# bibymaths/phoskintime

Measured on AMD Instinct MI355X. Metric: ODE-solve replicas/sec (32-state distributive, 14 tp), higher is better.
Workload: dtype f64

## Files before the change

### include/phoskin.h

```cpp
#ifndef PHOSKIN_H
#define PHOSKIN_H

#include <stdint.h>

#ifdef __cplusplus
extern "C" {
#endif

#define PK_VERSION 200

enum { PK_MODEL_DIST = 0, PK_MODEL_SUCC = 1, PK_MODEL_RAND = 2 };

enum {
  PK_METHOD_RODAS4 = 0,
  PK_METHOD_BDF2   = 1,
  PK_METHOD_RK4    = 2,
  PK_METHOD_LRP8   = 3,
  PK_METHOD_LRP12  = 5,
  PK_METHOD_DP5    = 4,
  PK_METHOD_ARK436 = 6,
  PK_METHOD_ROS34PW2 = 7
};

enum {
// ... 135 lines not shown
  const int32_t *p_prot, *t_prot; const double *obs_prot, *w_prot;
  const int32_t *p_rna, *t_rna;   const double *obs_rna, *w_rna;
  const int32_t *p_pho, *s_pho, *t_pho; const double *obs_pho, *w_pho;
  int32_t prot_base_idx, rna_base_idx, pho_base_idx;
} pk_loss_data;
typedef struct pk_loss pk_loss;
pk_loss* pk_network_loss_create(pk_ctx*, pk_net*, const pk_loss_data*, int T);
void     pk_network_loss_destroy(pk_loss*);
int      pk_network_objective_batch(pk_ctx*, pk_net*, pk_loss*, int64_t B, const double* Y, int T, int loss_mode,
                                    const double* x, int x_is_raw, const double* defaults, const double* lambdas, double fail_value,
                                    const int32_t* status, double* loss_sums, double* F);

int      pk_network_simulate_objective_batch(pk_ctx*, pk_net*, pk_loss*, int64_t B, const double* x, int x_is_raw, const double* y0,
                                             int y0_is_batched, const double* t_host, int T, const pk_solver_opts* opts, int loss_mode,
                                             const double* defaults, const double* lambdas, double fail_value, double* Y, int32_t* status,
                                             int32_t* n_steps, double* loss_sums, double* F);

int pk_loss_fn_batch_host(pk_ctx*, int combinatorial, int loss_mode, int64_t B, const double* Y, int T, int S, const pk_loss_data*,
                          const int32_t* prot_map, int N, double* loss_sums);

int pk_network_observables_batch(pk_ctx*, pk_net*, pk_loss*, int64_t B, const double* Y, int T, double eps, double* pred);

enum { PK_NET_METRIC_TOTAL_SIGNAL = 0, PK_NET_METRIC_MEAN = 1, PK_NET_METRIC_VARIANCE = 2, PK_NET_METRIC_L2_NORM = 3 };
int pk_network_simulate_measure_batch(pk_ctx*, pk_net*, pk_loss* lists, int64_t B, const double* x, int x_is_raw, const double* y0,
                                      int y0_is_batched, const double* t_host, int T, const pk_solver_opts* opts, double eps, int metric_id,
                                      double* Y, double* pred, double* metric, int32_t* status, int32_t* n_steps);

double pk_time_solve_protein_batch(pk_ctx*, int iters, int model, int n_sites, int64_t B,
                                   const double* theta, const double* y0, int y0_is_batched,
                                   const double* t, int T, const pk_solver_opts* opts,
                                   double* sol, double* flat, double* metric, int metric_id,
                                   int32_t* status, int32_t* n_steps);

double pk_measure_hbm_gbs(pk_ctx*, int64_t bytes, int iters);
double pk_measure_hbm_stream_gbs(pk_ctx*, int64_t bytes, int iters, int mode);
double pk_measure_fp64_fma_tflops(pk_ctx*, int iters);

#define PK_COMM_ID_BYTES 128
int pk_comm_unique_id(pk_ctx*, char* id_out );
int pk_comm_init(pk_ctx*, const char* id , int rank, int world);
int pk_comm_rank(pk_ctx*);
int pk_comm_world(pk_ctx*);
int pk_allgather_f64(pk_ctx*, const double* send, int64_t count, double* recv);
int pk_comm_destroy(pk_ctx*);

#ifdef __cplusplus
}
#endif
#endif
```

### phoskintime_amd/_capi.py

```python
from __future__ import annotations

import ctypes as C
import os
from pathlib import Path

_HERE = Path(__file__).resolve().parent
LIB_PATH = _HERE / "libphoskin_hip.so"

DIST, SUCC, RAND = 0, 1, 2
MODEL_IDS = {"distmod": DIST, "succmod": SUCC, "randmod": RAND}
MODEL_NAMES = {v: k for k, v in MODEL_IDS.items()}
METHOD_RODAS4, METHOD_BDF2, METHOD_RK4, METHOD_LRP8, METHOD_DP5, METHOD_LRP12, METHOD_ARK436, METHOD_ROS34PW2 = 0, 1, 2, 3, 4, 5, 6, 7
METHODS = {"rodas4": METHOD_RODAS4, "bdf2": METHOD_BDF2, "rk4": METHOD_RK4, "lrp8": METHOD_LRP8, "dp5": METHOD_DP5, "lrp12": METHOD_LRP12, "ark436": METHOD_ARK436, "ros34pw2": METHOD_ROS34PW2}
LINSOLVE_AUTO, LINSOLVE_DENSE, LINSOLVE_STRUCTURED = 0, 1, 2
LINSOLVES = {"auto": LINSOLVE_AUTO, "dense": LINSOLVE_DENSE, "structured": LINSOLVE_STRUCTURED}
KERNEL_AUTO, KERNEL_GROUP, KERNEL_TPR, KERNEL_WORKSPACE = 0, 1, 2, 3
KERNELS = {"auto": KERNEL_AUTO, "group": KERNEL_GROUP, "tpr": KERNEL_TPR, "workspace": KERNEL_WORKSPACE}
NORMS = {"default": 0, "max": 1, "rms": 2}
METRICS = {"total_signal": 0, "mean_activity": 1, "variance": 2, "dynamics": 3, "l2_norm": 4}
ST_NONFINITE, ST_MAXSTEPS, ST_HMIN = 1, 2, 4


class PhoskinLibraryError(RuntimeError):
    pass


class PhoskinError(RuntimeError):
    pass


class NetworkDesc(C.Structure):
    _fields_ = [("model", C.c_int32), ("N", C.c_int32), ("n_K", C.c_int32), ("total_sites", C.c_int32), ("n_grid", C.c_int32),
                ("offset_y", C.c_void_p), ("offset_s", C.c_void_p), ("n_sites", C.c_void_p),
                ("W_indptr", C.c_void_p), ("W_indices", C.c_void_p), ("W_data", C.c_void_p),
                ("TF_indptr", C.c_void_p), ("TF_indices", C.c_void_p), ("TF_data", C.c_void_p),
                ("tf_deg", C.c_void_p), ("driver_map", C.c_void_p), ("kin_grid", C.c_void_p), ("kin_Kmat", C.c_void_p)]


class LossData(C.Structure):
    _fields_ = [("n_prot", C.c_int32), ("n_rna", C.c_int32), ("n_pho", C.c_int32),
                ("p_prot", C.c_void_p), ("t_prot", C.c_void_p), ("obs_prot", C.c_void_p), ("w_prot", C.c_void_p),
                ("p_rna", C.c_void_p), ("t_rna", C.c_void_p), ("obs_rna", C.c_void_p), ("w_rna", C.c_void_p),
                ("p_pho", C.c_void_p), ("s_pho", C.c_void_p), ("t_pho", C.c_void_p), ("obs_pho", C.c_void_p), ("w_pho", C.c_void_p),
                ("prot_base_idx", C.c_int32), ("rna_base_idx", C.c_int32), ("pho_base_idx", C.c_int32)]


class SolverOpts(C.Structure):
    _fields_ = [("method", C.c_int32), ("linsolve", C.c_int32), ("rtol", C.c_double), ("atol", C.c_double),
                ("h0", C.c_double), ("rk4_h", C.c_double), ("max_steps", C.c_int32), ("clip_nonneg", C.c_int32),
                ("normalize", C.c_int32), ("stage_form", C.c_int32), ("kernel", C.c_int32), ("err_norm", C.c_int32)]


SYMBOLS = (
    "pk_version", "pk_create", "pk_create_error", "pk_destroy", "pk_last_error", "pk_set_stream", "pk_use_own_stream", "pk_synchronize", "pk_default_opts", "pk_workspace_stats",
    "pk_protein_n_states", "pk_protein_n_params", "pk_protein_flat_len",
    "pk_solve_protein_batch", "pk_solve_protein_sens_batch", "pk_protein_sens_available", "pk_rhs_protein_batch", "pk_jacobian_protein_batch", "pk_steady_state_protein_batch", "pk_morris_build_batch", "pk_morris_effects_batch", "pk_score_fit_batch",
    "pk_solve_protein_batch_host", "pk_solve_protein_sens_batch_host", "pk_rhs_protein_batch_host", "pk_jacobian_protein_batch_host",
    "pk_time_solve_protein_batch", "pk_measure_hbm_gbs", "pk_measure_hbm_stream_gbs", "pk_measure_fp64_fma_tflops",
    "pk_network_create", "pk_network_destroy", "pk_network_n_states", "pk_network_n_var",
    "pk_network_rhs_batch", "pk_network_jacobian_batch", "pk_network_unpack_batch", "pk_network_simulate_batch",
    "pk_network_loss_create", "pk_network_loss_destroy", "pk_network_objective_batch", "pk_network_simulate_objective_batch", "pk_network_observables_batch", "pk_network_simulate_measure_batch", "pk_frechet_batch", "pk_loss_fn_batch_host", "pk_network_resolve_method",
    "pk_network_workspace_bytes",
    "pk_comm_unique_id", "pk_comm_init", "pk_comm_rank", "pk_comm_world", "pk_allgather_f64", "pk_comm_destroy",
)

PK_OK, PK_ERR_ARG, PK_ERR_UNSUPPORTED, PK_ERR_HIP, PK_ERR_NOMEM = 0, -1, -2, -3, -4
NET_METRIC_TOTAL_SIGNAL, NET_METRIC_MEAN, NET_METRIC_VARIANCE, NET_METRIC_L2_NORM = 0, 1, 2, 3
NET_METRICS = {"total_signal": NET_METRIC_TOTAL_SIGNAL, "mean": NET_METRIC_MEAN, "variance": NET_METRIC_VARIANCE, "l2_norm": NET_METRIC_L2_NORM}

_lib = None


def load():
    global _lib
    if _lib is not None:
        return _lib
    import torch
    if not LIB_PATH.exists():
        raise PhoskinLibraryError(
            f"{LIB_PATH} not found: build it with `python -c 'import __graft_entry__ as g; g.build()'` "
            "(hipcc --offload-arch=gfx950). There is no CPU fallback.")
    try:
        lib = C.CDLL(str(LIB_PATH), mode=getattr(os, "RTLD_NOW", 2))
    except OSError as e:
        raise PhoskinLibraryError(f"cannot load {LIB_PATH}: {e}") from e
    vp, i32, i64, dbl = C.c_void_p, C.c_int, C.c_int64, C.c_double
    optp = C.POINTER(SolverOpts)
    lib.pk_version.restype = i32
    lib.pk_create.restype = vp; lib.pk_create.argtypes = [i32]
    lib.pk_create_error.restype = C.c_char_p; lib.pk_create_error.argtypes = []
# ... 24 lines not shown
    lib.pk_network_create.restype = vp; lib.pk_network_create.argtypes = [vp, C.POINTER(NetworkDesc)]
    lib.pk_network_destroy.restype = None; lib.pk_network_destroy.argtypes = [vp]
    lib.pk_network_n_states.restype = i32; lib.pk_network_n_states.argtypes = [vp]
    lib.pk_network_n_var.restype = i32; lib.pk_network_n_var.argtypes = [vp]
    for f in ("pk_network_rhs_batch", "pk_network_jacobian_batch"):
        getattr(lib, f).restype = i32; getattr(lib, f).argtypes = [vp, vp, i64, vp, i32, vp, i32, vp, i32, vp]
    lib.pk_network_simulate_batch.restype = i32
    lib.pk_network_simulate_batch.argtypes = [vp, vp, i64, vp, i32, vp, i32, vp, i32, optp, vp, vp, vp]
    lib.pk_network_loss_create.restype = vp; lib.pk_network_loss_create.argtypes = [vp, vp, C.POINTER(LossData), i32]
    lib.pk_network_loss_destroy.restype = None; lib.pk_network_loss_destroy.argtypes = [vp]
    lib.pk_network_objective_batch.restype = i32
    lib.pk_network_objective_batch.argtypes = [vp, vp, vp, i64, vp, i32, i32, vp, i32, vp, vp, dbl, vp, vp, vp]
    lib.pk_network_simulate_objective_batch.restype = i32
    lib.pk_network_simulate_objective_batch.argtypes = [vp, vp, vp, i64, vp, i32, vp, i32, vp, i32, optp, i32, vp, vp, dbl, vp, vp, vp, vp, vp]
    lib.pk_network_observables_batch.restype = i32
    lib.pk_network_observables_batch.argtypes = [vp, vp, vp, i64, vp, i32, dbl, vp]
    lib.pk_network_simulate_measure_batch.restype = i32
    lib.pk_network_simulate_measure_batch.argtypes = [vp, vp, vp, i64, vp, i32, vp, i32, vp, i32, optp, dbl, i32, vp, vp, vp, vp, vp]
    lib.pk_network_resolve_method.restype = i32; lib.pk_network_resolve_method.argtypes = [vp, optp]
    lib.pk_network_workspace_bytes.restype = i64; lib.pk_network_workspace_bytes.argtypes = [vp, vp, i64]
    lib.pk_loss_fn_batch_host.restype = i32
    lib.pk_loss_fn_batch_host.argtypes = [vp, i32, i32, i64, vp, i32, i32, C.POINTER(LossData), vp, i32, vp]
    lib.pk_network_unpack_batch.restype = i32; lib.pk_network_unpack_batch.argtypes = [vp, vp, i64, vp, vp]
    lib.pk_comm_unique_id.restype = i32; lib.pk_comm_unique_id.argtypes = [vp, C.c_char_p]
    lib.pk_comm_init.restype = i32; lib.pk_comm_init.argtypes = [vp, C.c_char_p, i32, i32]
    lib.pk_comm_rank.restype = i32; lib.pk_comm_rank.argtypes = [vp]
    lib.pk_comm_world.restype = i32; lib.pk_comm_world.argtypes = [vp]
    lib.pk_allgather_f64.restype = i32; lib.pk_allgather_f64.argtypes = [vp, vp, i64, vp]
    lib.pk_comm_destroy.restype = i32; lib.pk_comm_destroy.argtypes = [vp]
    lib.pk_score_fit_batch.restype = i32; lib.pk_score_fit_batch.argtypes = [vp, i64, vp, i32, vp, vp, i32, vp, vp]
    lib.pk_measure_hbm_gbs.restype = dbl; lib.pk_measure_hbm_gbs.argtypes = [vp, i64, i32]
    lib.pk_measure_hbm_stream_gbs.restype = dbl; lib.pk_measure_hbm_stream_gbs.argtypes = [vp, i64, i32, i32]
    lib.pk_measure_fp64_fma_tflops.restype = dbl; lib.pk_measure_fp64_fma_tflops.argtypes = [vp, i32]
    lib.pk_time_solve_protein_batch.restype = dbl
    lib.pk_time_solve_protein_batch.argtypes = [vp, i32] + solve_args[1:]
    _lib = lib
    return lib


def default_opts(**kw) -> SolverOpts:
    o = SolverOpts()
    load().pk_default_opts(C.byref(o))
    for k, v in kw.items():
        if v is None:
            continue
        if k == "method" and isinstance(v, str):
            v = METHODS[v]
        if k == "linsolve" and isinstance(v, str):
            v = LINSOLVES[v]
        if k == "kernel" and isinstance(v, str):
            v = KERNELS[v]
        if k == "err_norm" and isinstance(v, str):
            v = NORMS[v]
        if not hasattr(o, k):
            raise TypeError(f"unknown solver option {k!r}")
        setattr(o, k, v)
    return o


class Context:

    def __init__(self, device: int = 0):
        self.lib = load()
        self.device = int(device)
        self._h = self.lib.pk_create(self.device)
        if not self._h:
# ... 34 lines not shown
```

### phoskintime_amd/csrc/pk_capi.hip

```cpp
#include <hip/hip_runtime.h>
#include <cmath>
#include <cstdio>
#include <cstring>
#include <cstdlib>
#include <mutex>
#include <string>
#include "../../include/phoskin.h"
#include "pk_launch.hpp"
#include "pk_sens.hpp"

struct pk_arena {
  void* p = nullptr; size_t bytes = 0; long long allocs = 0;
};
struct pk_ctx {
  int device;
  hipStream_t own_stream;
  hipStream_t stream;
  std::string err;
  hipEvent_t ev0, ev1;
  pk_arena stage, scratch;
  void* pin = nullptr; size_t pin_bytes = 0; long long pin_allocs = 0;
  std::recursive_mutex mu;
  hipEvent_t scratch_ev = nullptr; bool scratch_used = false;
};
// ... 227 lines not shown
  }
  static const int level6_env = [] { const char* v = getenv("PK_RAND_LEVEL6"); return v ? atoi(v) : 0; }();
  if (model == PK_MODEL_RAND && n_sites == 6 && level6_env == 1 && o.method == PK_METHOD_LRP12 && !o.stage_form) {
    if (B > 0x7fffffffLL) return fail(c, PK_ERR_ARG, "batch too large for one launch");
    PK_HIP(c, hipSetDevice(c->device));
    PK_HIP(c, pk::launch_rand_level(a, c->stream));
    return PK_OK;
  }
  static const int parity56_env = [] { const char* v = getenv("PK_RAND_PARITY56"); return v ? atoi(v) : -1; }();
  if (model == PK_MODEL_RAND && ((n_sites == 6 && parity56_env != 0) || (n_sites == 5 && parity56_env == 1)) && o.method == PK_METHOD_LRP12 &&
      o.linsolve == PK_LINSOLVE_AUTO && !o.stage_form) {
    if (B > 0x7fffffffLL) return fail(c, PK_ERR_ARG, "batch too large for one launch");
    PK_HIP(c, hipSetDevice(c->device));
    PK_HIP(c, pk::launch_rand_parity(a, c->stream));
    return PK_OK;
  }
  const bool rand_fast = model == PK_MODEL_RAND && resolvent_method(o.method) && (o.linsolve == PK_LINSOLVE_AUTO || a.S > 64) && !o.stage_form;
  if (a.S > 64 && !rand_fast)
    return fail(c, PK_ERR_UNSUPPORTED, "randmod n_sites = 6 (S = 65): only method RODAS4 / LRP8 in resolvent form (the generic kernels hold one state per lane)");
  const int G = a.S > 64 ? 64 : group_width(a.S);
  const long long rpb = 256 / G;
  const long long nblk = (B + rpb - 1) / rpb;
  if (nblk > 0x7fffffffLL) return fail(c, PK_ERR_ARG, "batch too large for one launch");
  const bool structured = (o.linsolve != PK_LINSOLVE_DENSE) && (model != PK_MODEL_RAND);
  PK_HIP(c, hipSetDevice(c->device));
  dim3 grid((unsigned)nblk);
  static const int tpr_env_once = [] { const char* v = getenv("PK_TPR"); return v ? atoi(v) : -1; }();
  const int tpr_env = o.kernel == PK_KERNEL_GROUP ? 0 : o.kernel == PK_KERNEL_TPR ? 1 : tpr_env_once;
  const long long tpr_min = (model == PK_MODEL_SUCC) ? (n_sites <= 8 ? 16384 : 32768) : (model == PK_MODEL_RAND) ? 32768 : (n_sites <= 8 ? 32768 : 49152);
  const bool tpr = o.method == PK_METHOD_LRP12 && o.linsolve == PK_LINSOLVE_AUTO && !o.stage_form && pk::tpr_available(model, n_sites) &&
                   (tpr_env == 1 || (tpr_env != 0 && B >= tpr_min));
  if (tpr)
    PK_HIP(c, pk::launch_tpr(a, model, c->stream));
  else if (model == PK_MODEL_DIST && resolvent_method(o.method) && o.linsolve == PK_LINSOLVE_AUTO && !o.stage_form)
    pk::launch_dist_fast(a, o.method, c->stream);
  else if (rand_fast)
    pk::launch_rand_fast(a, o.method, c->stream);
  else
    kSolve[model][gidx(G)](a, o.method, structured, grid, c->stream);
  PK_HIP(c, hipGetLastError());
  return PK_OK;
}

int pk_rhs_protein_batch(pk_ctx* c, int model, int n_sites, int64_t B, const double* theta, const double* y, double* dydt) {
  if (!c) return PK_ERR_ARG;
  int rc = check_model(c, model, n_sites);
  if (rc) return rc;
  if (B < 0) return fail(c, PK_ERR_ARG, "B must be >= 0");
  if (B == 0) return PK_OK;
  if (!theta || !y || !dydt) return fail(c, PK_ERR_ARG, "null pointer");
  const int S = pk::n_states(model, n_sites), P = pk::n_params(model, n_sites), G = S > 64 ? 1 : group_width(S);
  const long long rpb = 256 / G, nblk = (S > 64 ? (B * S + 255) / 256 : (B + rpb - 1) / rpb);
  if (nblk > 0x7fffffffLL) return fail(c, PK_ERR_ARG, "batch too large for one launch");
  PK_HIP(c, hipSetDevice(c->device));
  dim3 grid((unsigned)nblk);
  if (S > 64 && model != PK_MODEL_RAND) pk::launch_chain_rhs_wide(model, theta, y, dydt, (long long)B, n_sites, S, P, c->stream);
  else if (S > 64) pk::launch_rand_rhs_wide(theta, y, dydt, (long long)B, n_sites, S, P, c->stream);
  else kRhs[model][gidx(G)](theta, y, dydt, (long long)B, n_sites, S, P, grid, c->stream);
  PK_HIP(c, hipGetLastError());
  return PK_OK;
}

int pk_jacobian_protein_batch(pk_ctx* c, int model, int n_sites, int64_t B, const double* theta, double* J) {
  if (!c) return PK_ERR_ARG;
  int rc = check_model(c, model, n_sites);
  if (rc) return rc;
  if (B < 0) return fail(c, PK_ERR_ARG, "B must be >= 0");
  if (B == 0) return PK_OK;
  if (!theta || !J) return fail(c, PK_ERR_ARG, "null pointer");
// ... 164 lines not shown
  if (!c) return PK_ERR_ARG;
  std::lock_guard<std::recursive_mutex> host_guard(c->mu);
  int rc = check_model(c, model, n_sites);
  if (rc) return rc;
  if (B < 0) return fail(c, PK_ERR_ARG, "B must be >= 0");
  if (B == 0) return PK_OK;
  if (!theta || !y || !dydt) return fail(c, PK_ERR_ARG, "null pointer");
  const size_t S = pk::n_states(model, n_sites), P = pk::n_params(model, n_sites);
  PK_HIP(c, hipSetDevice(c->device));
  HostCall h(c);
  const size_t o_th = h.add_in(theta, (size_t)B * P * 8), o_y = h.add_in(y, (size_t)B * S * 8), o_f = h.add_out(dydt, (size_t)B * S * 8);
  if ((rc = h.upload())) return rc;
  rc = pk_rhs_protein_batch(c, model, n_sites, B, h.dev<const double>(o_th), h.dev<const double>(o_y), h.dev<double>(o_f));
  if (rc) { (void)hipStreamSynchronize(c->stream); return rc; }
  return h.download();
}

int pk_jacobian_protein_batch_host(pk_ctx* c, int model, int n_sites, int64_t B, const double* theta, double* J) {
  if (!c) return PK_ERR_ARG;
  std::lock_guard<std::recursive_mutex> host_guard(c->mu);
  int rc = check_model(c, model, n_sites);
  if (rc) return rc;
  if (B < 0) return fail(c, PK_ERR_ARG, "B must be >= 0");
  if (B == 0) return PK_OK;
  if (!theta || !J) return fail(c, PK_ERR_ARG, "null pointer");
  const size_t S = pk::n_states(model, n_sites), P = pk::n_params(model, n_sites);
  PK_HIP(c, hipSetDevice(c->device));
  HostCall h(c);
  const size_t o_th = h.add_in(theta, (size_t)B * P * 8), o_J = h.add_out(J, (size_t)B * S * S * 8);
  if ((rc = h.upload())) return rc;
  rc = pk_jacobian_protein_batch(c, model, n_sites, B, h.dev<const double>(o_th), h.dev<double>(o_J));
  if (rc) { (void)hipStreamSynchronize(c->stream); return rc; }
  return h.download();
}

double pk_time_solve_protein_batch(pk_ctx* c, int iters, int model, int n_sites, int64_t B, const double* theta,
                                   const double* y0, int y0_is_batched, const double* t, int T,
                                   const pk_solver_opts* opts, double* sol, double* flat, double* metric, int metric_id,
                                   int32_t* status, int32_t* n_steps) {
  if (!c || iters < 1) return -1.0;
  if (hipSetDevice(c->device) != hipSuccess) return -1.0;
  if (hipEventRecord(c->ev0, c->stream) != hipSuccess) return -1.0;
  for (int i = 0; i < iters; ++i) {
    int rc = pk_solve_protein_batch(c, model, n_sites, B, theta, y0, y0_is_batched, t, T, opts, sol, flat, metric, metric_id, status, n_steps);
    if (rc) return (double)rc;
  }
  if (hipEventRecord(c->ev1, c->stream) != hipSuccess) return -1.0;
  if (hipEventSynchronize(c->ev1) != hipSuccess) { c->err = "hipEventSynchronize failed"; return -1.0; }
  float ms = 0.f;
  if (hipEventElapsedTime(&ms, c->ev0, c->ev1) != hipSuccess) return -1.0;
  return (double)ms / iters;
}

}

namespace pk {
__global__ __launch_bounds__(256) void score_fit_kernel(const double* __restrict__ theta, const int P, const double* __restrict__ target,
                                                        const double* __restrict__ pred, const int N, const long long B,
                                                        const double alpha, const double beta, const double gamma, const double delta,
                                                        const double mu, double* __restrict__ out) {
  const long long b = (long long)blockIdx.x * 4 + (threadIdx.x >> 6);
  if (b >= B) return;
  const int lane = threadIdx.x & 63;
  const double* pb = pred + b * N;
  double s1 = 0.0, s2 = 0.0;
  for (int k = lane; k < N; k += 64) { const double r = fabs(target[k] - pb[k]) / (double)N; s1 += r; s2 = __builtin_fma(r, r, s2); }
// ... 26 lines not shown
```

### phoskintime_amd/csrc/pk_dist_fast.hpp

```cpp
#pragma once
#include "pk_solve_kernel.hpp"

namespace pk {

template <int RPL, bool RES = false>
struct Stg {
  double s[RPL];
  double R, P;
};
template <int RPL>
struct Stg<RPL, true> {
  double s[RPL];
};
template <int RPL, bool RES>
__device__ __forceinline__ void trk_axpy(Stg<RPL, RES>& acc, const double a, const Stg<RPL, RES>& u) {
#pragma unroll
  for (int j = 0; j < RPL; ++j) acc.s[j] = __builtin_fma(a, u.s[j], acc.s[j]);
  if constexpr (!RES) {
    acc.R = __builtin_fma(a, u.R, acc.R);
    acc.P = __builtin_fma(a, u.P, acc.P);
  }
}
template <int RPL, bool RES>
__device__ __forceinline__ Stg<RPL, RES> trk_scale(const double a, const Stg<RPL, RES>& u) {
// ... 30 lines not shown
  __host__ __device__ static __forceinline__ bool normalize(const SolveArgs& A) { return A.normalize != 0; }
  __host__ __device__ static __forceinline__ bool flat(const SolveArgs& A) { return A.flat != nullptr; }
  __host__ __device__ static __forceinline__ bool sol(const SolveArgs& A) { return A.sol != nullptr; }
  __host__ __device__ static __forceinline__ int mclass(const SolveArgs& A) { return dist_metric_class(A); }
  static bool matches(const SolveArgs&) { return true; }
};
using DistSolSum = DistFixed<true, false, false, true, PK_DM_SUM>;
using DistSolOnly = DistFixed<true, false, false, true, PK_DM_NONE>;
using DistFlatOnly = DistFixed<true, false, true, false, PK_DM_NONE>;

template <int RPL, int MC, bool RES = false> constexpr int dist_fast_slots() {
  return MC == PK_DM_FULL ? 3 * RPL + (RES ? 4 : 6) : MC == PK_DM_SUM ? 2 * RPL + 1 : 2 * RPL;
}

template <int RPL, bool PARK, int NT> struct Parked;
template <int RPL, int NT> struct Parked<RPL, false, NT> {
  double v[3 * RPL + 6];
  __device__ __forceinline__ explicit Parked(double*) {}
  template <int K> __device__ __forceinline__ double get() const { return v[K]; }
  template <int K> __device__ __forceinline__ void set(double x) { v[K] = x; }
  __device__ __forceinline__ void fence() {}
};
template <int RPL, int NT> struct Parked<RPL, true, NT> {
  typedef __attribute__((address_space(3))) double lds_double;
  lds_double* base;
  __device__ __forceinline__ explicit Parked(double* lds) : base((lds_double*)lds + threadIdx.x) {}
  template <int K> __device__ __forceinline__ double get() const { return base[K * NT]; }
  template <int K> __device__ __forceinline__ void set(double x) { base[K * NT] = x; }
  __device__ __forceinline__ void fence() { asm volatile("" : "+v"(base)); }
};
template <int RPL, bool PARK, int NT = 256, class CFG = DistAny, bool RES = false>
constexpr size_t dist_fast_lds_bytes() { return PARK ? (size_t)(dist_fast_slots<RPL, CFG::SLOT_MC, RES>() + RPL) * NT * sizeof(double) : 0; }

template <int G, int RPL, int METHOD, bool PARK = false, int MINB = (PARK ? 2 : 1), int NT = 256, class CFG = DistAny, bool RES = false>
__global__ __launch_bounds__(NT, MINB) void dist_fast_kernel(const SolveArgs A) {
  using Tab = ResolventTab<METHOD>;
  using Vec = Stg<RPL, RES>;
  extern __shared__ __align__(16) double park_lds[];
  Parked<RPL, PARK, NT> pk(park_lds);
  static_assert(dist_fast_lds_bytes<RPL, PARK, 64, CFG, RES>() * 4 * MINB <= 160 * 1024, "parked slots exceed the CU's LDS at this occupancy");
  constexpr int MCS = CFG::SLOT_MC;
  constexpr int NSL = dist_fast_slots<RPL, MCS, RES>(), FB = 3 * RPL + (RES ? 0 : 2);
  constexpr int K_SR = 0, K_DG = RPL, K_PS = 2 * RPL, K_PR = 3 * RPL, K_PP = 3 * RPL + 1, K_M1 = (MCS == PK_DM_FULL ? FB : 2 * RPL),
                K_M2 = FB + 1, K_MD = FB + 2, K_SH = FB + 3, K_Y = NSL;
  constexpr int RPB = NT / G;
  const int lane = lane_id();
  const int l = threadIdx.x & (G - 1);
  const long long rep = (long long)blockIdx.x * RPB + (threadIdx.x / G);
  if (rep >= A.B) return;
  const int n = A.n_sites, S = A.S, T = A.T;
  const int mclass = CFG::mclass(A);
  const double* __restrict__ th = A.theta + rep * A.P;

  const double cA = th[0], cB = th[1], cC = th[2];
  const bool isR = RES && l == 0, isP = RES && l == 1;
  const double w0 = isR ? cC : 1.0, k3 = isR ? cA : 0.0;
  double lsum = 0.0;
  static_for<RPL>([&](auto jc) {
    constexpr int j = decltype(jc)::value;
    const int i = l + G * j - (RES ? 2 : 0);
    const bool ok = i >= 0 && i < n;
    const double sr = ok ? th[4 + i] : 0.0;
    double dg = ok ? 1.0 + th[4 + n + i] : 1.0;
    if constexpr (RES && j == 0) dg = isR ? cB : isP ? -cC : dg;
    pk.template set<K_SR + j>(sr);
    pk.template set<K_DG + j>(dg);
    lsum += sr;
  });
  const double Dsum = th[3] + gsum<G>(lsum, lane);
  auto sites_only = [&](const double (&s)[RPL]) {
// ... 101 lines not shown
            const double dR = vR - prevR, dP = vP - prevP;
            mdyn = __builtin_fma(dR, dR, mdyn); mdyn = __builtin_fma(dP, dP, mdyn);
          }
          pk.template set<K_PR>(vR); pk.template set<K_PP>(vP);
        }
        pk.template set<K_M2>(m2); pk.template set<K_MD>(mdyn);
      }
    }
  };
  auto finish = [&](const int status, const int acc, const int rej) {
    if (mclass != PK_DM_NONE) {
      const double L = 2.0 * T + (double)T * n;
      const double tot = gsum<G>(pk.template get<K_M1>(), lane);
      double m = tot;
      if (A.metric_id == PK_METRIC_MEAN_ACTIVITY) m = tot / L;
      if constexpr (MCS == PK_DM_FULL) if (mclass == PK_DM_FULL) {
        const double m2 = pk.template get<K_M2>(), mdyn = pk.template get<K_MD>(), shift = pk.template get<K_SH>();
        switch (A.metric_id) {
          case PK_METRIC_VARIANCE: { const double q = gsum<G>(m2, lane); const double ms = tot / L - shift; m = q / L - ms * ms; } break;
          case PK_METRIC_DYNAMICS: m = gsum<G>(mdyn, lane); break;
          default: { const double q = gsum<G>(m2, lane); m = sqrt(fmax(q + 2.0 * shift * tot - L * shift * shift, 0.0)); } break;
        }
      }
      if (l == 0) A.metric[rep] = m;
    }
    if (l == 0) {
      if (A.status) A.status[rep] = status;
      if (A.n_steps) { A.n_steps[2 * rep] = acc; A.n_steps[2 * rep + 1] = rej; }
    }
  };

  emit(0, y, std::false_type{});
  int status = PK_ST_OK, nacc = 0;
  if (T < 2) { finish(status, 0, 0); return; }

  const double rtol = A.rtol, atol = A.atol;
  auto q = [&](double e, double ya, double yb) { return fabs(e) * approx_rcp(__builtin_fma(rtol, fmax(fabs(ya), fabs(yb)), atol)); };
  auto group_max = [&](const Vec& num, const Vec& a, const Vec& b) {
    auto mx = [](double p, double r) { return (p > r || p != p) ? p : r; };
    double m;
    if constexpr (RES) m = q(num.s[0], a.s[0], b.s[0]); else m = mx(q(num.R, a.R, b.R), q(num.P, a.P, b.P));
#pragma unroll
    for (int j = (RES ? 1 : 0); j < RPL; ++j) m = mx(m, q(num.s[j], a.s[j], b.s[j]));
    return gmax<G>(m, lane);
  };
  auto err_norm = [&](const Vec& e, const Vec& y, const Vec& yn) {
    constexpr int X = RES ? 0 : 2;
    double r[RPL + X];
    if constexpr (!RES) { r[0] = q(e.R, y.R, yn.R); r[1] = q(e.P, y.P, yn.P); }
    static_for<RPL>([&](auto jc) {
      constexpr int j = decltype(jc)::value;
      r[X + j] = q(e.s[j], y.s[j], yn.s[j]);
    });
    double m = tree_max(r);
    if (any_nan(r)) m = __builtin_inf();
    return gmax_num<G>(m, lane);
  };
  auto rhs_of = [&](const Vec& Y, const double sg) {
    Vec f;
    if constexpr (RES) {
      const double Rb = bcast<G, 0>(Y.s[0]), Pb = bcast<G, 1>(Y.s[0]);
      static_for<RPL>([&](auto jc) {
        constexpr int j = decltype(jc)::value;
        const double sr = pk.template get<K_SR + j>(), dg = pk.template get<K_DG + j>();
        if constexpr (j == 0) f.s[0] = __builtin_fma(isP ? -Dsum : sr, Pb, __builtin_fma(-dg, isP ? Rb : Y.s[0], isP ? sg : k3));
        else f.s[j] = __builtin_fma(sr, Pb, -dg * Y.s[j]);
      });
// ... 89 lines not shown
      for (int j = 0; j < RPL; ++j) u.s[j] = __builtin_fma(cw[j], xP, t[j]);
      u.R = xR; u.P = xP;
    }
    return u;
  };

  bool after_reject = false;
  auto state_bad = [&]() {
    double rows[RPL];
#pragma unroll
    for (int j = 0; j < RPL; ++j) rows[j] = y.s[j];
    if constexpr (PARK) {
      pk.fence();
      static_for<RPL>([&](auto jc) { constexpr int j = decltype(jc)::value; rows[j] = pk.template get<K_Y + j>(); });
    }
    bool b;
    if constexpr (RES) b = ((isR || isP) && nonfinite(rows[0])) || nonfinite(sites_only(rows));
    else b = (nonfinite(y.R)) || (nonfinite(y.P)) || (nonfinite(site_sum<G>(rows, lane)));
    return gmax<G>(b ? 1.0 : 0.0, lane);
  };
  auto coef_bad = [&]() {
    if constexpr (RES) {
      long long r2 = rep;
      asm volatile("" : "+v"(r2));
      const double* t2 = A.theta + r2 * A.P;
      return (nonfinite(t2[0])) || (nonfinite(t2[1])) || (nonfinite(t2[2]));
    } else return (nonfinite(cA)) || (nonfinite(cB)) || (nonfinite(cC));
  };
  int nsec = 0;
  __builtin_amdgcn_s_waitcnt(0x0F70);
  while (true) {
    bool nonfin = false;
    while (true) {
      const double tnx = A.t[k + 1 < T ? k + 1 : T - 1];
      const bool over = (CFG::LITERAL ? nacc + nsec : nsec) >= A.max_steps;
      const bool last = (tc + 1.0001 * h >= te);
      const double hs = last ? te - tc : ((tc + 2.0 * h > te) ? 0.5 * (te - tc) : h);
      if (over || !(hs > 1e-14 * fmax(fabs(tc), 1e-3))) { status |= over ? PK_ST_MAXSTEPS : PK_ST_HMIN; break; }
      if constexpr (PARK) {
        pk.fence();
        static_for<RPL>([&](auto jc) { constexpr int j = decltype(jc)::value; y.s[j] = pk.template get<K_Y + j>(); });
      }
      factor(Tab::GAM * hs);

      Vec z;
      {
        Vec r = y;
        if constexpr (RES) r.s[0] = __builtin_fma(qq, k3, y.s[0]); else r.R = __builtin_fma(qq, cA, y.R);
        z = solve(r);
        trk_axpy(z, -1.0, y);
      }
      Vec yn = y; trk_axpy(yn, Tab::B[0] / Tab::GAM, z);
      Vec u6;
      static_for<Tab::NS - 1>([&](auto kc) {
        constexpr int kk = 1 + decltype(kc)::value;
        constexpr double bk = Tab::B[kk] / Tab::GAM, ek = Tab::E[kk] / Tab::GAM;
        z = solve(z);
        trk_axpy(yn, bk, z);
        if constexpr (kk == 1) u6 = trk_scale(ek, z); else trk_axpy(u6, ek, z);
      });

      double err;
      if constexpr (CFG::LITERAL) err = group_max(u6, y, yn); else err = err_norm(u6, y, yn);
      const bool acc = (err <= 1.0);
      if constexpr (PARK) {
        if (acc) {
// ... 18 lines not shown
          continue;
        }
      } else {
        ++nsec;
        if (__builtin_expect(err != err || err > 1e300, 0)) { after_reject = true; h = 0.1 * hs; nonfin = true; break; }
      }
      double fac = root_q(err, Tab::Q) * (1.0 / 0.9);
      fac = fmax(1.0 / 6.0, fmin(5.0, fac));
      double hnew = hs * fast_rcp(fac);
      const bool land = acc && last;
      if constexpr (CFG::LITERAL) { nacc += acc ? 1 : 0; nsec += acc ? 0 : 1; }
      else nacc += (int)acc;
      if (acc && after_reject) hnew = fmin(hnew, hs);
      after_reject = !acc;
      if constexpr (CFG::LITERAL) tc = land ? te : (acc ? tc + hs : tc);
      h = (land && hs < h) ? fmax(hnew, h) : hnew;
      if (land) {
        if constexpr (!CFG::LITERAL) tc = te;
        te = tnx;
        asm volatile("" : "+v"(te));
        emit(k, y, std::false_type{});
        ++k;
      }
      if (k >= T) break;
    }
    if (CFG::LITERAL || !nonfin) break;
    if (state_bad() != 0.0 || coef_bad() || (nonfinite(Dsum)) || (nonfinite(Scw))) {
      status |= PK_ST_NONFINITE; break;
    }
  }
  const int nrej = CFG::LITERAL ? nsec : nsec - nacc;
  if (status != PK_ST_OK)
    for (; k < T; ++k) emit(k, y, std::true_type{});
  finish(status, nacc, nrej);
}

}
```

### phoskintime_amd/csrc/pk_dist_fast12.hpp

```cpp
#pragma once
#include "pk_dist_fast.hpp"
#include "pk_launch.hpp"

namespace pk {

template <int G, int RPL, bool PARK, int NT, class CFG, bool RES>
static void launch_cfg(const SolveArgs& a, hipStream_t st) {
  const long long rpb = NT / G;
  const long long nblk = (a.B + rpb - 1) / rpb;
  constexpr size_t lds = dist_fast_lds_bytes<RPL, PARK, NT, CFG, RES>();
  auto kern = dist_fast_kernel<G, RPL, PK_METHOD_LRP12, PARK, (PARK ? 2 : 1), NT, CFG, RES>;
  if constexpr (lds > 48 * 1024) {
    static const bool once = [kern] {
      (void)hipFuncSetAttribute((const void*)kern, hipFuncAttributeMaxDynamicSharedMemorySize, (int)lds);
      return true;
    }();
    (void)once;
  }
  hipLaunchKernelGGL(kern, dim3((unsigned)nblk), dim3(NT), lds, st, a);
}

template <int G, int RPL, bool PARK, int NT, bool RES>
static void launch_nt(const SolveArgs& a, hipStream_t st) {
  if (DistSolSum::matches(a)) launch_cfg<G, RPL, PARK, NT, DistSolSum, RES>(a, st);
  else if (DistSolOnly::matches(a)) launch_cfg<G, RPL, PARK, NT, DistSolOnly, RES>(a, st);
  else if (DistFlatOnly::matches(a)) launch_cfg<G, RPL, PARK, NT, DistFlatOnly, RES>(a, st);
  else launch_cfg<G, RPL, PARK, NT, DistAny, RES>(a, st);
}

void launch_dist_fast12_resident(const SolveArgs& a, bool wg256, hipStream_t st);

}
```

### phoskintime_amd/csrc/pk_inst_dist_fast12.hip

```cpp
#include "pk_dist_fast12.hpp"
#include <cstdio>
#include <cstdlib>
#include <cstring>

namespace pk {

template <int G, int RPL>
static void launch_plain(const SolveArgs& a, hipStream_t st) { launch_nt<G, RPL, false, 256, false>(a, st); }

template <int G, int RPL>
static void launch_parked(const SolveArgs& a, hipStream_t st) { launch_nt<G, RPL, true, 64, false>(a, st); }

void launch_dist_fast12(const SolveArgs& a, hipStream_t st) {
  const int n = a.n_sites;
  static const bool force84 = getenv("PK_DIST_LAYOUT") && !strcmp(getenv("PK_DIST_LAYOUT"), "8x4");
  static const bool wg256 = getenv("PK_DIST_LAYOUT") && !strcmp(getenv("PK_DIST_LAYOUT"), "wg256");
  static const bool shadow = getenv("PK_DIST_LAYOUT") && !strcmp(getenv("PK_DIST_LAYOUT"), "shadow");
  const int slots = n <= 32 ? 4 * ((n + 3) / 4) : 8 * ((n + 7) / 8);
  if (!shadow && !(force84 && n > 16 && n <= 32) && n >= 1 && slots >= n + 2) { launch_dist_fast12_resident(a, wg256, st); return; }
  if (n <= 4) launch_plain<4, 1>(a, st);
  else if (n <= 8) launch_plain<4, 2>(a, st);
  else if (n <= 12) launch_plain<4, 3>(a, st);
  else if (n <= 16) launch_plain<4, 4>(a, st);
  else if (n <= 32 && force84) launch_plain<8, 4>(a, st);
  else if (n <= 20) launch_parked<4, 5>(a, st);
  else if (n <= 24) launch_parked<4, 6>(a, st);
  else if (n <= 28) launch_parked<4, 7>(a, st);
  else if (n <= 32 && wg256) launch_nt<4, 8, true, 256, false>(a, st);
  else if (n <= 32) launch_parked<4, 8>(a, st);
  else if (n <= 40) launch_parked<8, 5>(a, st);
  else if (n <= 48) launch_parked<8, 6>(a, st);
  else if (n <= 56) launch_parked<8, 7>(a, st);
  else launch_parked<8, 8>(a, st);
}

}
```

### phoskintime_amd/csrc/pk_inst_dist_fast12r.hip

```cpp
#include "pk_dist_fast12.hpp"

namespace pk {

void launch_dist_fast12_resident(const SolveArgs& a, bool wg256, hipStream_t st) {
  const int n = a.n_sites;
  if (n <= 2) launch_nt<4, 1, false, 256, true>(a, st);
  else if (n <= 6) launch_nt<4, 2, false, 256, true>(a, st);
  else if (n <= 10) launch_nt<4, 3, false, 256, true>(a, st);
  else if (n <= 14) launch_nt<4, 4, false, 256, true>(a, st);
  else if (n <= 18) launch_nt<4, 5, true, 64, true>(a, st);
  else if (n <= 22) launch_nt<4, 6, true, 64, true>(a, st);
  else if (n <= 26) launch_nt<4, 7, true, 64, true>(a, st);
  else if (n <= 30 && wg256) launch_nt<4, 8, true, 256, true>(a, st);
  else if (n <= 30) launch_nt<4, 8, true, 64, true>(a, st);
  else if (n <= 38) launch_nt<8, 5, true, 64, true>(a, st);
  else if (n <= 46) launch_nt<8, 6, true, 64, true>(a, st);
  else if (n <= 54) launch_nt<8, 7, true, 64, true>(a, st);
  else launch_nt<8, 8, true, 64, true>(a, st);
}

}
```

### phoskintime_amd/csrc/pk_launch.hpp

```cpp
#pragma once
#include "pk_solve_kernel.hpp"

namespace pk {

using SolveLauncher = void (*)(const SolveArgs&, int method, bool structured, dim3 grid, hipStream_t);
using RhsLauncher = void (*)(const double* theta, const double* y, double* dydt, long long B, int n, int S, int P, dim3 grid, hipStream_t);
using JacLauncher = void (*)(const double* theta, double* J, long long B, int n, int S, int P, dim3 grid, hipStream_t);
using SteadyLauncher = void (*)(const double* theta, double* yss, int32_t* status, long long B, int n, int S, int P, dim3 grid, hipStream_t);

#define PK_DECL(M, G)                                                                                     \
  void launch_solve_m##M##_g##G(const SolveArgs&, int, bool, dim3, hipStream_t);                           \
  void launch_rhs_m##M##_g##G(const double*, const double*, double*, long long, int, int, int, dim3, hipStream_t); \
  void launch_jac_m##M##_g##G(const double*, double*, long long, int, int, int, dim3, hipStream_t);          \
  void launch_steady_m##M##_g##G(const double*, double*, int32_t*, long long, int, int, int, dim3, hipStream_t);
PK_DECL(0, 8) PK_DECL(0, 16) PK_DECL(0, 32) PK_DECL(0, 64)
PK_DECL(1, 8) PK_DECL(1, 16) PK_DECL(1, 32) PK_DECL(1, 64)
PK_DECL(2, 8) PK_DECL(2, 16) PK_DECL(2, 32) PK_DECL(2, 64)
#undef PK_DECL

void launch_dist_fast(const SolveArgs&, int method, hipStream_t);
void launch_rand_fast(const SolveArgs&, int method, hipStream_t);
bool tpr_available(int model, int n_sites);
hipError_t launch_tpr(const SolveArgs&, int model, hipStream_t);
struct SensArgs;
bool sens_available(int model, int n_sites);
hipError_t launch_sens(const SensArgs&, int model, hipStream_t);
bool wide_chain_fits(int S, int n_sites);
hipError_t launch_wide_chain(const SolveArgs&, int model, hipStream_t);
bool rand_dense_available(int n_sites);
hipError_t launch_rand_dense(const SolveArgs&, hipStream_t);
hipError_t launch_rand_level(const SolveArgs&, hipStream_t);
hipError_t launch_rand_parity(const SolveArgs&, hipStream_t, bool pinned_family = false);
bool wide_rand_in_lds(int n_sites);
size_t wide_rand_scratch_bytes(int n_sites, long long B);
hipError_t launch_wide_rand(const SolveArgs&, double* scratch, hipStream_t);
hipError_t launch_wide_steady(int model, const double* theta, double* yss, int32_t* status, long long B, int n, int S, int P, hipStream_t);
void launch_chain_rhs_wide(int model, const double* theta, const double* y, double* dydt, long long B, int n, int S, int P, hipStream_t);
void launch_chain_jac_wide(int model, const double* theta, double* J, long long B, int n, int S, int P, hipStream_t);
void launch_rand_rhs_wide(const double* theta, const double* y, double* dydt, long long B, int n, int S, int P, hipStream_t);
void launch_rand_jac_wide(const double* theta, double* J, long long B, int n, int S, int P, hipStream_t);

}
```

### phoskintime_amd/csrc/pk_solve_kernel.hpp

```cpp
#pragma once
#include <hip/hip_runtime.h>
#include <cstdint>
#include "../../include/phoskin.h"
#include "pk_linsolve.hpp"

namespace pk {

struct SolveArgs {
  const double* theta; const double* y0; const double* t;
  double* sol; double* flat; double* metric; int32_t* status; int32_t* n_steps;
  long long B; int n_sites; int S; int P; int T; int F; int n_obs; int y0_batched; int metric_id;
  double rtol, atol, h0, rk4_h; int max_steps; int clip; int normalize; int stage_form;
};

namespace r4 {
constexpr double GAM = 0.25;
constexpr double A21 = 0.1544000000000000e+01, A31 = 0.9466785280815826e+00, A32 = 0.2557011698983284e+00;
constexpr double A41 = 0.3314825187068521e+01, A42 = 0.2896124015972201e+01, A43 = 0.9986419139977817e+00;
constexpr double A51 = 0.1221224509226641e+01, A52 = 0.6019134481288629e+01, A53 = 0.1253708332932087e+02, A54 = -0.6878860361058950e+00;
constexpr double C21 = -0.5668800000000000e+01, C31 = -0.2430093356833875e+01, C32 = -0.2063599157091915e+00;
constexpr double C41 = -0.1073529058151375e+00, C42 = -0.9594562251023355e+01, C43 = -0.2047028614809616e+02;
constexpr double C51 = 0.7496443313967647e+01, C52 = -0.1024680431464352e+02, C53 = -0.3399990352819905e+02, C54 = 0.1170890893206160e+02;
constexpr double C61 = 0.8083246795921522e+01, C62 = -0.7981132988064893e+01, C63 = -0.3152159432874371e+02, C64 = 0.1631930543123136e+02, C65 = -0.6058818238834054e+01;
constexpr double RB1 = 0.25, RB2 = -0.30261563040255475781, RB3 = 2.0437958549435498747, RB4 = -1.1490271157486588988,
                 RB5 = 0.12712918827688397052, RB6 = 0.030717702930779034113;
constexpr double RE2 = -0.27896255898136486925, RE3 = 0.80616997401331598084, RE4 = -0.74473456815175834943,
                 RE5 = 0.18680945018902833694, RE6 = 0.030717702930779034113;
}

template <int METHOD> struct ResolventTab;
template <> struct ResolventTab<PK_METHOD_RODAS4> {
  static constexpr int NS = 6;
  static constexpr double GAM = 0.25;
  static constexpr double Q = 4.0;
  static constexpr double B[6] = {r4::RB1, r4::RB2, r4::RB3, r4::RB4, r4::RB5, r4::RB6};
  static constexpr double E[6] = {0.0, r4::RE2, r4::RE3, r4::RE4, r4::RE5, r4::RE6};
};
template <> struct ResolventTab<PK_METHOD_LRP8> {
  static constexpr int NS = 8;
  static constexpr double GAM = 0.22;
  static constexpr double Q = 7.0;
  static constexpr double B[8] = {0.22, 0.896963014494355498137, -4.05804045796110421602, 10.5343409578260650281,
                                  -11.197471732915163878, 6.15403680296552740685, -1.75732530837770792816, 0.207496723968028089083};
  static constexpr double E[8] = {0.0, 0.207496723968028089083, -1.2449803438081685345, 3.11245085952042133624,
                                  -4.14993447936056178166, 3.11245085952042133624, -1.2449803438081685345, 0.207496723968028089083};
// ... 326 lines not shown
```

Before: 232.9 million.

## Add wave-priority pacing for tail-heavy dist LRP12 grids plus block tracing

For the parked 64-thread LRP12 distributive kernel, the launcher computes how many blocks fit at once across the device. When the grid is only slightly larger than that, it turns on a default scheduling mode. First-wave leader blocks get top wave priority, and the other waves lower their priority as they move through the time points. The aim is to let the long-running first-wave blocks finish sooner, so the tail of the grid overlaps better. The change also adds an optional trace variant behind an environment variable that records per-block timestamps and hardware IDs, plus an env-var override for the schedule. This costs extra ballot and setprio instructions in the step loop and can hurt when the wrong waves get priority.

```diff
diff --git a/include/phoskin.h b/include/phoskin.h
--- a/include/phoskin.h
+++ b/include/phoskin.h
@@ -191,6 +191,10 @@
                                    double* sol, double* flat, double* metric, int metric_id,
                                    int32_t* status, int32_t* n_steps);
 
+int         pk_dist_sched_parse(const char* value);
+const char* pk_dist_sched_names(void);
+int         pk_dist_trace_set(pk_ctx*, void* records, int64_t capacity);
+
 double pk_measure_hbm_gbs(pk_ctx*, int64_t bytes, int iters);
 double pk_measure_hbm_stream_gbs(pk_ctx*, int64_t bytes, int iters, int mode);
 double pk_measure_fp64_fma_tflops(pk_ctx*, int iters);
diff --git a/phoskintime_amd/_capi.py b/phoskintime_amd/_capi.py
--- a/phoskintime_amd/_capi.py
+++ b/phoskintime_amd/_capi.py
@@ -56,6 +56,7 @@
     "pk_protein_n_states", "pk_protein_n_params", "pk_protein_flat_len",
     "pk_solve_protein_batch", "pk_solve_protein_sens_batch", "pk_protein_sens_available", "pk_rhs_protein_batch", "pk_jacobian_protein_batch", "pk_steady_state_protein_batch", "pk_morris_build_batch", "pk_morris_effects_batch", "pk_score_fit_batch",
     "pk_solve_protein_batch_host", "pk_solve_protein_sens_batch_host", "pk_rhs_protein_batch_host", "pk_jacobian_protein_batch_host",
+    "pk_dist_sched_parse", "pk_dist_sched_names", "pk_dist_trace_set",
     "pk_time_solve_protein_batch", "pk_measure_hbm_gbs", "pk_measure_hbm_stream_gbs", "pk_measure_fp64_fma_tflops",
     "pk_network_create", "pk_network_destroy", "pk_network_n_states", "pk_network_n_var",
     "pk_network_rhs_batch", "pk_network_jacobian_batch", "pk_network_unpack_batch", "pk_network_simulate_batch",
@@ -146,6 +147,9 @@
     lib.pk_measure_hbm_gbs.restype = dbl; lib.pk_measure_hbm_gbs.argtypes = [vp, i64, i32]
     lib.pk_measure_hbm_stream_gbs.restype = dbl; lib.pk_measure_hbm_stream_gbs.argtypes = [vp, i64, i32, i32]
     lib.pk_measure_fp64_fma_tflops.restype = dbl; lib.pk_measure_fp64_fma_tflops.argtypes = [vp, i32]
+    lib.pk_dist_sched_parse.restype = i32; lib.pk_dist_sched_parse.argtypes = [C.c_char_p]
+    lib.pk_dist_sched_names.restype = C.c_char_p; lib.pk_dist_sched_names.argtypes = []
+    lib.pk_dist_trace_set.restype = i32; lib.pk_dist_trace_set.argtypes = [vp, vp, i64]
     lib.pk_time_solve_protein_batch.restype = dbl
     lib.pk_time_solve_protein_batch.argtypes = [vp, i32] + solve_args[1:]
     _lib = lib
diff --git a/phoskintime_amd/csrc/pk_capi.hip b/phoskintime_amd/csrc/pk_capi.hip
--- a/phoskintime_amd/csrc/pk_capi.hip
+++ b/phoskintime_amd/csrc/pk_capi.hip
@@ -283,9 +283,10 @@
                    (tpr_env == 1 || (tpr_env != 0 && B >= tpr_min));
   if (tpr)
     PK_HIP(c, pk::launch_tpr(a, model, c->stream));
-  else if (model == PK_MODEL_DIST && resolvent_method(o.method) && o.linsolve == PK_LINSOLVE_AUTO && !o.stage_form)
+  else if (model == PK_MODEL_DIST && resolvent_method(o.method) && o.linsolve == PK_LINSOLVE_AUTO && !o.stage_form) {
+    if (pk::dist_sched_env() < 0) return fail(c, PK_ERR_ARG, std::string("PK_DIST_SCHED must be one of: ") + pk::kDistSchedNames);
     pk::launch_dist_fast(a, o.method, c->stream);
-  else if (rand_fast)
+  } else if (rand_fast)
     pk::launch_rand_fast(a, o.method, c->stream);
   else
     kSolve[model][gidx(G)](a, o.method, structured, grid, c->stream);
@@ -516,6 +517,19 @@
   rc = pk_jacobian_protein_batch(c, model, n_sites, B, h.dev<const double>(o_th), h.dev<double>(o_J));
   if (rc) { (void)hipStreamSynchronize(c->stream); return rc; }
   return h.download();
+}
+
+int pk_dist_sched_parse(const char* value) { return pk::dist_sched_parse(value); }
+
+const char* pk_dist_sched_names(void) { return pk::kDistSchedNames; }
+
+int pk_dist_trace_set(pk_ctx* c, void* records, int64_t capacity) {
+  if (!c) return PK_ERR_ARG;
+  if (capacity < 0 || (records && capacity < 1)) return fail(c, PK_ERR_ARG, "capacity must be >= 1 with a buffer");
+  PK_HIP(c, hipSetDevice(c->device));
+  PK_HIP(c, hipStreamSynchronize(c->stream));
+  PK_HIP(c, pk::dist_trace_set(records, (long long)capacity));
+  return PK_OK;
 }
 
 double pk_time_solve_protein_batch(pk_ctx* c, int iters, int model, int n_sites, int64_t B, const double* theta,
diff --git a/phoskintime_amd/csrc/pk_dist_fast.hpp b/phoskintime_amd/csrc/pk_dist_fast.hpp
--- a/phoskintime_amd/csrc/pk_dist_fast.hpp
+++ b/phoskintime_amd/csrc/pk_dist_fast.hpp
@@ -86,10 +86,57 @@
 template <int RPL, bool PARK, int NT = 256, class CFG = DistAny, bool RES = false>
 constexpr size_t dist_fast_lds_bytes() { return PARK ? (size_t)(dist_fast_slots<RPL, CFG::SLOT_MC, RES>() + RPL) * NT * sizeof(double) : 0; }
 
-template <int G, int RPL, int METHOD, bool PARK = false, int MINB = (PARK ? 2 : 1), int NT = 256, class CFG = DistAny, bool RES = false>
+enum { PK_DSCHED_OFF = 0, PK_DSCHED_LEAD_SLOT = 1, PK_DSCHED_LEVEL = 2, PK_DSCHED_LEAD_BLOCK = 4 };
+constexpr int PK_DSCHED_K2 = 5, PK_DSCHED_K1 = 9;
+constexpr int PK_HWREG_HW_ID = 4 | (31 << 11), PK_HWREG_HW_ID_WAVE = 4 | (3 << 11), PK_HWREG_XCC_ID = 20 | (31 << 11);
+
+struct DistTraceRec {
+  unsigned long long t_entry, t_exit;
+  unsigned block, hw_id, xcc_id, iters;
+};
+struct DistTraceBuf { DistTraceRec* rec; long long capacity; };
+template <int TRACE> struct DistTrace;
+
+template <int G, int RPL, int METHOD, bool PARK = false, int MINB = (PARK ? 2 : 1), int NT = 256, class CFG = DistAny, bool RES = false, int TRACE = 0>
 __global__ __launch_bounds__(NT, MINB) void dist_fast_kernel(const SolveArgs A) {
   using Tab = ResolventTab<METHOD>;
   using Vec = Stg<RPL, RES>;
+  constexpr bool PACE = PARK && NT == 64 && METHOD == PK_METHOD_LRP12;
+  static_assert(!TRACE || NT == 64, "the trace holds one record per workgroup: one wave each");
+  if constexpr (TRACE) {
+    const unsigned long long t0 = __builtin_amdgcn_s_memrealtime();
+    const DistTraceBuf tb = DistTrace<TRACE>::get();
+    if (threadIdx.x == 0 && tb.rec && (long long)blockIdx.x < tb.capacity) {
+      DistTraceRec* r = tb.rec + blockIdx.x;
+      r->t_entry = t0; r->t_exit = 0; r->block = blockIdx.x; r->iters = 0;
+      r->hw_id = __builtin_amdgcn_s_getreg(PK_HWREG_HW_ID); r->xcc_id = __builtin_amdgcn_s_getreg(PK_HWREG_XCC_ID);
+    }
+  }
+  int witer = 0;
+  auto trace_exit = [&]() {
+    if constexpr (TRACE) {
+      int it = witer;
+      for (int o = 32; o > 0; o >>= 1) { const int v = __shfl_xor(it, o); it = v > it ? v : it; }
+      const DistTraceBuf tb = DistTrace<TRACE>::get();
+      if (threadIdx.x == 0 && tb.rec && (long long)blockIdx.x < tb.capacity) {
+        DistTraceRec* r = tb.rec + blockIdx.x;
+        r->iters = (unsigned)it; r->t_exit = __builtin_amdgcn_s_memrealtime();
+      }
+    }
+  };
+  bool paced = false;
+  if constexpr (PACE) {
+    const int sched = A.sched;
+    if (sched != PK_DSCHED_OFF) {
+      bool leader = false;
+      if ((int)gridDim.x > A.R1) {
+        if (sched & PK_DSCHED_LEAD_SLOT) leader = (int)blockIdx.x < A.R1 && __builtin_amdgcn_s_getreg(PK_HWREG_HW_ID_WAVE) == 0;
+        if (sched & PK_DSCHED_LEAD_BLOCK) leader = leader || (int)blockIdx.x < A.R1 / 3;
+      }
+      if (leader) __builtin_amdgcn_s_setprio(3);
+      paced = !leader && (sched & PK_DSCHED_LEVEL) != 0;
+    }
+  }
   extern __shared__ __align__(16) double park_lds[];
   Parked<RPL, PARK, NT> pk(park_lds);
   static_assert(dist_fast_lds_bytes<RPL, PARK, 64, CFG, RES>() * 4 * MINB <= 160 * 1024, "parked slots exceed the CU's LDS at this occupancy");
@@ -257,7 +304,7 @@
 
   emit(0, y, std::false_type{});
   int status = PK_ST_OK, nacc = 0;
-  if (T < 2) { finish(status, 0, 0); return; }
+  if (T < 2) { trace_exit(); finish(status, 0, 0); return; }
 
   const double rtol = A.rtol, atol = A.atol;
   auto q = [&](double e, double ya, double yb) { return fabs(e) * approx_rcp(__builtin_fma(rtol, fmax(fabs(ya), fabs(yb)), atol)); };
@@ -413,6 +460,12 @@
   while (true) {
     bool nonfin = false;
     while (true) {
+      if constexpr (TRACE) ++witer;
+      if constexpr (PACE) if (paced) {
+        if (__builtin_amdgcn_ballot_w64(k < PK_DSCHED_K2) != 0) __builtin_amdgcn_s_setprio(2);
+        else if (__builtin_amdgcn_ballot_w64(k < PK_DSCHED_K1) != 0) __builtin_amdgcn_s_setprio(1);
+        else __builtin_amdgcn_s_setprio(0);
+      }
       const double tnx = A.t[k + 1 < T ? k + 1 : T - 1];
       const bool over = (CFG::LITERAL ? nacc + nsec : nsec) >= A.max_steps;
       const bool last = (tc + 1.0001 * h >= te);
@@ -497,6 +550,7 @@
   const int nrej = CFG::LITERAL ? nsec : nsec - nacc;
   if (status != PK_ST_OK)
     for (; k < T; ++k) emit(k, y, std::true_type{});
+  trace_exit();
   finish(status, nacc, nrej);
 }
 
diff --git a/phoskintime_amd/csrc/pk_dist_fast12.hpp b/phoskintime_amd/csrc/pk_dist_fast12.hpp
--- a/phoskintime_amd/csrc/pk_dist_fast12.hpp
+++ b/phoskintime_amd/csrc/pk_dist_fast12.hpp
@@ -4,12 +4,17 @@
 
 namespace pk {
 
-template <int G, int RPL, bool PARK, int NT, class CFG, bool RES>
+constexpr int PK_DSCHED_UNSET = 0x100;
+int dist_sched_parse(const char* v);
+int dist_sched_env();
+extern const char* const kDistSchedNames;
+
+template <int G, int RPL, bool PARK, int NT, class CFG, bool RES, int TRACE = 0>
 static void launch_cfg(const SolveArgs& a, hipStream_t st) {
   const long long rpb = NT / G;
   const long long nblk = (a.B + rpb - 1) / rpb;
   constexpr size_t lds = dist_fast_lds_bytes<RPL, PARK, NT, CFG, RES>();
-  auto kern = dist_fast_kernel<G, RPL, PK_METHOD_LRP12, PARK, (PARK ? 2 : 1), NT, CFG, RES>;
+  auto kern = dist_fast_kernel<G, RPL, PK_METHOD_LRP12, PARK, (PARK ? 2 : 1), NT, CFG, RES, TRACE>;
   if constexpr (lds > 48 * 1024) {
     static const bool once = [kern] {
       (void)hipFuncSetAttribute((const void*)kern, hipFuncAttributeMaxDynamicSharedMemorySize, (int)lds);
@@ -17,7 +22,24 @@
     }();
     (void)once;
   }
-  hipLaunchKernelGGL(kern, dim3((unsigned)nblk), dim3(NT), lds, st, a);
+  if constexpr (PARK && NT == 64) {
+    static const int resident = [kern] {
+      int dev = 0, cus = 0, per_cu = 0;
+      if (hipGetDevice(&dev) != hipSuccess || hipDeviceGetAttribute(&cus, hipDeviceAttributeMultiprocessorCount, dev) != hipSuccess ||
+          hipOccupancyMaxActiveBlocksPerMultiprocessor(&per_cu, (const void*)kern, NT, lds) != hipSuccess || per_cu < 1 || cus < 1) {
+        (void)hipGetLastError();
+        return 0x7fffffff;
+      }
+      return per_cu * cus;
+    }();
+    SolveArgs b = a;
+    const int env = dist_sched_env();
+    const bool pays = G == 4 && nblk <= (long long)resident + resident / 3;
+    b.sched = env == PK_DSCHED_UNSET ? (pays ? PK_DSCHED_LEAD_SLOT | PK_DSCHED_LEVEL : PK_DSCHED_OFF) : env < 0 ? (int)PK_DSCHED_OFF : env;
+    b.R1 = resident;
+    hipLaunchKernelGGL(kern, dim3((unsigned)nblk), dim3(NT), lds, st, b);
+  } else
+    hipLaunchKernelGGL(kern, dim3((unsigned)nblk), dim3(NT), lds, st, a);
 }
 
 template <int G, int RPL, bool PARK, int NT, bool RES>
@@ -29,5 +51,7 @@
 }
 
 void launch_dist_fast12_resident(const SolveArgs& a, bool wg256, hipStream_t st);
+void launch_dist_fast12_traced(const SolveArgs& a, hipStream_t st);
+hipError_t dist_trace_set(void* records, long long capacity);
 
 }
diff --git a/phoskintime_amd/csrc/pk_inst_dist_fast12.hip b/phoskintime_amd/csrc/pk_inst_dist_fast12.hip
--- a/phoskintime_amd/csrc/pk_inst_dist_fast12.hip
+++ b/phoskintime_amd/csrc/pk_inst_dist_fast12.hip
@@ -4,6 +4,34 @@
 #include <cstring>
 
 namespace pk {
+
+const char* const kDistSchedNames = "off, lead, level, lead+level";
+
+int dist_sched_parse(const char* v) {
+  if (!v || !*v) return -1;
+  if (!strcmp(v, "off")) return PK_DSCHED_OFF;
+  int bits = 0;
+  for (const char* p = v; *p;) {
+    const char* e = strchr(p, '+');
+    const size_t len = e ? (size_t)(e - p) : strlen(p);
+    auto is = [&](const char* w) { return strlen(w) == len && !strncmp(p, w, len); };
+    int b;
+    if (is("lead") || is("lead:slot")) b = PK_DSCHED_LEAD_SLOT;
+    else if (is("lead:block")) b = PK_DSCHED_LEAD_BLOCK;
+    else if (is("level")) b = PK_DSCHED_LEVEL;
+    else return -1;
+    if (bits & b) return -1;
+    bits |= b;
+    p += len;
+    if (e) { ++p; if (!*p) return -1; }
+  }
+  return bits;
+}
+
+int dist_sched_env() {
+  static const int v = [] { const char* e = getenv("PK_DIST_SCHED"); return e ? dist_sched_parse(e) : PK_DSCHED_UNSET; }();
+  return v;
+}
 
 template <int G, int RPL>
 static void launch_plain(const SolveArgs& a, hipStream_t st) { launch_nt<G, RPL, false, 256, false>(a, st); }
diff --git a/phoskintime_amd/csrc/pk_inst_dist_fast12r.hip b/phoskintime_amd/csrc/pk_inst_dist_fast12r.hip
--- a/phoskintime_amd/csrc/pk_inst_dist_fast12r.hip
+++ b/phoskintime_amd/csrc/pk_inst_dist_fast12r.hip
@@ -1,9 +1,13 @@
 #include "pk_dist_fast12.hpp"
+#include <cstdlib>
+#include <cstring>
 
 namespace pk {
 
 void launch_dist_fast12_resident(const SolveArgs& a, bool wg256, hipStream_t st) {
   const int n = a.n_sites;
+  static const bool traced = getenv("PK_DIST_TRACE") && !strcmp(getenv("PK_DIST_TRACE"), "1");
+  if (traced && n > 26 && n <= 30 && !wg256 && DistSolSum::matches(a)) { launch_dist_fast12_traced(a, st); return; }
   if (n <= 2) launch_nt<4, 1, false, 256, true>(a, st);
   else if (n <= 6) launch_nt<4, 2, false, 256, true>(a, st);
   else if (n <= 10) launch_nt<4, 3, false, 256, true>(a, st);
diff --git a/phoskintime_amd/csrc/pk_inst_dist_fast12t.hip b/phoskintime_amd/csrc/pk_inst_dist_fast12t.hip
--- /dev/null
+++ b/phoskintime_amd/csrc/pk_inst_dist_fast12t.hip
@@ -0,0 +1,17 @@
+#include "pk_dist_fast12.hpp"
+
+namespace pk {
+
+__device__ DistTraceBuf g_dist_trace = {nullptr, 0};
+template <> struct DistTrace<1> {
+  static __device__ __forceinline__ DistTraceBuf get() { return g_dist_trace; }
+};
+
+void launch_dist_fast12_traced(const SolveArgs& a, hipStream_t st) { launch_cfg<4, 8, true, 64, DistSolSum, true, 1>(a, st); }
+
+hipError_t dist_trace_set(void* records, long long capacity) {
+  const DistTraceBuf b = {(DistTraceRec*)records, records ? capacity : 0};
+  return hipMemcpyToSymbol(HIP_SYMBOL(g_dist_trace), &b, sizeof(b));
+}
+
+}
diff --git a/phoskintime_amd/csrc/pk_launch.hpp b/phoskintime_amd/csrc/pk_launch.hpp
--- a/phoskintime_amd/csrc/pk_launch.hpp
+++ b/phoskintime_amd/csrc/pk_launch.hpp
@@ -19,6 +19,10 @@
 #undef PK_DECL
 
 void launch_dist_fast(const SolveArgs&, int method, hipStream_t);
+int dist_sched_parse(const char* v);
+int dist_sched_env();
+extern const char* const kDistSchedNames;
+hipError_t dist_trace_set(void* records, long long capacity);
 void launch_rand_fast(const SolveArgs&, int method, hipStream_t);
 bool tpr_available(int model, int n_sites);
 hipError_t launch_tpr(const SolveArgs&, int model, hipStream_t);
diff --git a/phoskintime_amd/csrc/pk_solve_kernel.hpp b/phoskintime_amd/csrc/pk_solve_kernel.hpp
--- a/phoskintime_amd/csrc/pk_solve_kernel.hpp
+++ b/phoskintime_amd/csrc/pk_solve_kernel.hpp
@@ -11,6 +11,7 @@
   double* sol; double* flat; double* metric; int32_t* status; int32_t* n_steps;
   long long B; int n_sites; int S; int P; int T; int F; int n_obs; int y0_batched; int metric_id;
   double rtol, atol, h0, rk4_h; int max_steps; int clip; int normalize; int stage_form;
+  int sched = 0; int R1 = 0;
 };
 
 namespace r4 {
```

Result: faster. 241.0 million, median of 6 (+3.5%).
